# vkit-x/vkit

Hardware: AMD Instinct MI355X
Metric: Mpixels/s (2048^2 RGB, geo+photo chain) (higher is better)
Workload: dtype u8; 1 GPU; C3 fused chain: camera_cubic_curve remap (level 5) + gaussian_blur(sigma=1.0) + color_shift(37) + gaussion_noise(std=10.0, the numpy stream default_rng(5000 + i) drawn on the device inside every step), states built from the configs inside every step, 2048x2048x3 uint8, batch 256 per GPU; batch_per_gpu=256, image=2048x2048x3, noise_mode=tiles, states=built on the device from the configs inside every step (vkx_camera_states_dev), lanes=1

## Files before the change

### vkit_amd/csrc/fused.hip

```cpp
#include "vkx_internal.h"
#include "vkx_cell.h"
#include "vkx_color.h"

#include <float.h>
#include <memory>
#include <stdlib.h>
#include <string.h>

namespace {

constexpr int W = 64;
constexpr int RMAX = 3;
constexpr int NLDSCELL = 64;
#ifndef VKX_FUSED_NWAVES
#define VKX_FUSED_NWAVES 8
#endif
constexpr int NWAVES = VKX_FUSED_NWAVES;
constexpr int NTHREADS = 64 * NWAVES;
constexpr int ROWS_PER_WAVE = 8;
constexpr int WH = NWAVES * ROWS_PER_WAVE;
__host__ __device__ constexpr int tile_side(int R) { return (W - 2 * R) & ~3; }
__host__ __device__ constexpr int tile_height(int R) { return WH == W ? tile_side(R) : WH - 2 * R; }
#ifndef VKX_FUSED_CGROUP
#define VKX_FUSED_CGROUP 2
// ... 198 lines not shown
    }
    double r = __builtin_amdgcn_rcp(sdx);
    double e = fma(-sdx, r, 1.0);
    r = fma(r, e, r);
    e = fma(-sdx, r, 1.0);
    r = fma(r, e, r);
    const double snx = __builtin_amdgcn_div_scale(nx, de, true, &fnx);
    const double sny = __builtin_amdgcn_div_scale(ny, de, true, &fny);
    const double px = snx * r, py = sny * r;
    const double ex = fma(-sdx, px, snx), ey = fma(-sdx, py, sny);
    qx = __builtin_amdgcn_div_fixup(__builtin_amdgcn_div_fmas(ex, r, px, fnx), de, nx);
    qy = __builtin_amdgcn_div_fixup(__builtin_amdgcn_div_fmas(ey, r, py, fny), de, ny);
}

__device__ __forceinline__ bool div_pair_f32_fast(double nx, double ny, double de, float &fx, float &fy)
{
    double r = __builtin_amdgcn_rcp(de);
    double e = fma(-de, r, 1.0);
    r = fma(r, e, r);
    e = fma(-de, r, 1.0);
    r = fma(r, e, r);
    const double qx = nx * r, qy = ny * r;
    const uint32_t lx = (uint32_t)__double_as_longlong(qx) & 0x1fffffffu, ly = (uint32_t)__double_as_longlong(qy) & 0x1fffffffu;
    const bool danger = (lx - (0x10000000u - 16u)) < 32u || (ly - (0x10000000u - 16u)) < 32u;
    fx = (float)qx;
    fy = (float)qy;
    return __builtin_amdgcn_ballot_w64(danger) == 0;
}

__device__ __forceinline__ void rim_sample_rgb(gsrc_t src, int sh, int sw, ptrdiff_t sstride, int X, int Y, uint32_t &prb, uint32_t &pg)
{
    const int sx = vkd::sat_short(X >> 5), sy = vkd::sat_short(Y >> 5);
    const int fx = X & 31, fy = Y & 31;
    prb = 0; pg = 0;
    if (sx >= sw || sx + 1 < 0 || sy >= sh || sy + 1 < 0) return;
    const bool x0 = sx >= 0, x1 = sx + 1 < sw, y0 = sy >= 0, y1 = sy + 1 < sh;
    const gsrc_t r0 = src + (ptrdiff_t)sy * sstride + (ptrdiff_t)sx * 3, r1 = r0 + sstride;
    const int w00 = (32 - fy) * (32 - fx), w01 = (32 - fy) * fx, w10 = fy * (32 - fx), w11 = fy * fx;
    uint32_t c[3];
#pragma unroll
    for (int k = 0; k < 3; k++) {
        const int v0 = (x0 && y0) ? r0[k] : 0;
        const int v1 = (x1 && y0) ? r0[3 + k] : 0;
        const int v2 = (x0 && y1) ? r1[k] : 0;
        const int v3 = (x1 && y1) ? r1[3 + k] : 0;
        c[k] = (uint32_t)(v0 * w00 + v1 * w01 + v2 * w10 + v3 * w11 + 512) >> 10;
    }
    prb = c[0] | (c[2] << 16);
    pg = c[1];
}

struct HsvLut {
    int sdiv[256];
    int hdiv[256];
};

__device__ __forceinline__ void hue_shift_px(const int *sdiv, const int *hdiv, int delta, int &r, int &g, int &b)
{
    int H, S, V;
    vkd::rgb2hsv_full<true>(sdiv, hdiv, r, g, b, H, S, V);
    H = (H + delta) & 255;
    vkd::hsv2rgb_full(H, S, V, r, g, b);
}

constexpr int P_ = 97;
constexpr int kPairPitch = 2 * P_;
constexpr size_t kLdsOwn = sizeof(uint32_t) * WH * P_;
constexpr size_t kLdsHbB = 1024;
constexpr size_t kLdsCellR = sizeof(CellR) * NLDSCELL;
constexpr size_t kLdsCellH = sizeof(double) * 9 * NLDSCELL;
constexpr size_t kLdsLut = sizeof(int) * 512;
constexpr size_t kLdsSel = sizeof(uint32_t) * 8;
constexpr size_t kLdsNoiseRows = sizeof(uint32_t) * 2 * WH;
constexpr size_t kFusedLds = kLdsOwn + kLdsHbB + kLdsCellR + kLdsCellH + kLdsLut + kLdsSel + 16 + kLdsNoiseRows;

typedef const double __attribute__((address_space(3))) *lds_cdouble_t;


__device__ __forceinline__ int cvt_i32_sat(float v)
{
    int r;
    asm("v_cvt_i32_f32 %0, %1" : "=v"(r) : "v"(v));
    return r;
}

template <int KIND, bool STREAK = false, int RC = -1>
__device__ __forceinline__ void chain_tile(const ItemDev &it, const int tx, const int ty,
                                           const vkc::CellC *__restrict__ cells, const TileBin &bin,
                                           const HsvLut *__restrict__ lut, int phase_limit, const ElemPack *els = nullptr)
{
    constexpr bool INTERIOR = KIND == 1, EMPTY = KIND == 2;
    extern __shared__ __attribute__((aligned(16))) unsigned char smem[];
    uint32_t *own = (uint32_t *)smem;
    uint16_t *hbB = (uint16_t *)(smem + kLdsOwn);
    CellR *lcr = (CellR *)(smem + kLdsOwn + kLdsHbB);
    double *lch = (double *)(smem + kLdsOwn + kLdsHbB + kLdsCellR);
    int *lsdiv = (int *)(smem + kLdsOwn + kLdsHbB + kLdsCellR + kLdsCellH);
    int *lhdiv = lsdiv + 256;
    uint32_t *lsel = (uint32_t *)(lhdiv + 256);
    int *lflag = (int *)(lsel + 8);
    uint32_t *lnrow = (uint32_t *)(smem + kLdsOwn + kLdsHbB + kLdsCellR + kLdsCellH + kLdsLut + kLdsSel + 16);

    const int tid = threadIdx.x, lane = tid & 63, wave = __builtin_amdgcn_readfirstlane(tid >> 6);
    const int R = RC >= 0 ? RC : it.R, K = 2 * R + 1, Tw = tile_side(R), Th = tile_height(R);
    const int dw = it.dw, dh = it.dh;
    const int x0 = tx * Tw, y0 = ty * Th;
    const int tw = INTERIOR ? Tw : min(Tw, dw - x0), th = INTERIOR ? Th : min(Th, dh - y0);
    const int wx0 = x0 - R, wy0 = y0 - R;
    const int cx0 = INTERIOR ? wx0 : max(wx0, 0), cx1 = INTERIOR ? wx0 + W : min(wx0 + W, dw);
    const int cy0 = INTERIOR ? wy0 : max(wy0, 0), cy1 = INTERIOR ? wy0 + WH : min(wy0 + WH, dh);

    const gsrc_t src = (gsrc_t)it.src;
    const ptrdiff_t sstride = it.sstride;
    const int sh = it.sh, sw = it.sw;

    const int ocx = lane - R;
    const bool ocol = ocx >= 0 && ocx < tw;
    const int r0 = bin.rmin, c0 = bin.cmin;
    const int nr = max(0, bin.rmax1 - bin.rmin), ncol = max(0, bin.cmax1 - bin.cmin);
    const int nc = bin.rmax1 > 0 ? nr * ncol : 0;
    const int cw = it.cols - 1;
    const vkc::CellC *gcell = cells + it.cell_base;

    constexpr int kRecPerLane = NLDSCELL / (NTHREADS / 16);
    static_assert(NLDSCELL == kRecPerLane * (NTHREADS / 16), "whole records per lane and chunk");
    const float rcp_ncol = __builtin_amdgcn_rcpf((float)max(ncol, 1));
    auto chunk_fetch = [&](int base, int cn_, unsigned long long (&v)[kRecPerLane]) {
#pragma unroll
        for (int h = 0; h < kRecPerLane; h++) {
            const int rec = (tid >> 4) + h * (NTHREADS / 16);
            v[h] = 0;
            if (rec < cn_) {
                const int k = base + rec;
                const int rr = div_small(k, ncol, rcp_ncol), cc = k - rr * ncol;
                const unsigned long long VKX_GLOBAL *s8 =
                    (const unsigned long long VKX_GLOBAL *)(gcell + (r0 + rr) * cw + (c0 + cc));
                v[h] = s8[tid & 15];
            }
        }
    };
    auto chunk_store = [&](int cn_, const unsigned long long (&v)[kRecPerLane]) {
#pragma unroll
        for (int h = 0; h < kRecPerLane; h++) {
            const int rec = (tid >> 4) + h * (NTHREADS / 16), part = tid & 15;
            if (rec < cn_) {
                if (part < 8) ((unsigned long long *)(lch + rec * 9))[part] = v[h];
                else if (part < 15) ((unsigned long long *)(lcr + rec))[part - 8] = v[h];
            }
        }
    };
    auto load_chunk = [&](int base, int cn_) {
        unsigned long long v[kRecPerLane];
        chunk_fetch(base, cn_, v);
        chunk_store(cn_, v);
    };

    typedef uint32_t u32x2 __attribute__((ext_vector_type(2)));
    u32x2 nrec = {0u, 0u};
    const bool nrows_here = !(KIND == 3) && wave < WH / 64 && it.noise_rows != nullptr;
    const int nrow_y = wave * 64 + lane;
    if (nrows_here && nrow_y < th)
        nrec = ((const u32x2 VKX_GLOBAL *)it.noise_rows)[(size_t)(y0 + nrow_y) * (size_t)it.tiles_x + (size_t)tx];

    uint32_t kq[2 * RMAX + 1];
#pragma unroll
    for (int i = 0; i < 2 * RMAX + 1; i++) kq[i] = (R > 0 && i < K) ? it.kq[i < K - 1 - i ? i : K - 1 - i] : 0;
// ... 298 lines not shown
                ta[u] = 0; tb[u] = 0;
                if (fast[u]) {
                    const uint32_t o0 = __umul24((uint32_t)sy, (uint32_t)sstride) + __umul24((uint32_t)sx, 3u);
                    ta[u] = *(const u64_u1 VKX_GLOBAL *)(src + (size_t)o0);
                    tb[u] = *(const u64_u1 VKX_GLOBAL *)(src + (size_t)(o0 + (uint32_t)sstride));
                }
            }
            uint32_t prb[CGROUP], pg[CGROUP];
#pragma unroll
            for (int u = 0; u < CGROUP; u++) {
                prb[u] = 0; pg[u] = 0;
                if (!rowok[u]) continue;
                if (colok) {
                    const int fx = X[u] & 31, fy = Y[u] & 31;
                    if (fast[u]) {
                        const uint32_t wx = (uint32_t)(32 - fx) | ((uint32_t)fx << 24);
                        const uint32_t t0 = (uint32_t)ta[u], t1 = (uint32_t)(ta[u] >> 32), b0 = (uint32_t)tb[u], b1 = (uint32_t)(tb[u] >> 32);
                        const uint32_t ar = __builtin_amdgcn_udot4(t0, wx, 0u, false);
                        const uint32_t ag = __builtin_amdgcn_udot4(__builtin_amdgcn_alignbyte(t1, t0, 1), wx, 0u, false);
                        const uint32_t ab = __builtin_amdgcn_udot4(__builtin_amdgcn_alignbyte(t1, t0, 2), wx, 0u, false);
                        const uint32_t br = __builtin_amdgcn_udot4(b0, wx, 0u, false);
                        const uint32_t bg = __builtin_amdgcn_udot4(__builtin_amdgcn_alignbyte(b1, b0, 1), wx, 0u, false);
                        const uint32_t bb = __builtin_amdgcn_udot4(__builtin_amdgcn_alignbyte(b1, b0, 2), wx, 0u, false);
                        const uint32_t wy0 = (uint32_t)(32 - fy), wy1 = (uint32_t)fy;
                        const uint32_t r = mad_u24(br, wy1, mad_u24_cs(ar, wy0, 512u)) >> 10;
                        const uint32_t g = mad_u24(bg, wy1, mad_u24_cs(ag, wy0, 512u)) >> 10;
                        const uint32_t b = mad_u24(bb, wy1, mad_u24_cs(ab, wy0, 512u)) >> 10;
                        prb[u] = r | (b << 16);
                        pg[u] = g;
                    } else {
                        rim_sample_rgb(src, sh, sw, sstride, X[u], Y[u], prb[u], pg[u]);
                    }
                }
            }
            static_assert(CGROUP == 2, "phase D works on the window-row pair of one iteration");
            const int ly0 = wave * ROWS_PER_WAVE + g0;
            if (!(rowok[0] || rowok[1])) continue;
            if (R > 0) {
                const uint32_t gg = pg[0] | (pg[1] << 16);
                uint32_t a0 = 0, a1 = 0, ag = 0;
#pragma unroll
                for (int i = 0; i < 2 * RMAX + 1; i++) {
                    if (i < K) {
                        uint32_t v0 = prb[0], v1 = prb[1], vg = gg;
                        if (!(INTERIOR && RC >= 0 && i == RC)) {
                            v0 = (uint32_t)__builtin_amdgcn_ds_bpermute(srcl[i], (int)prb[0]);
                            v1 = (uint32_t)__builtin_amdgcn_ds_bpermute(srcl[i], (int)prb[1]);
                            vg = (uint32_t)__builtin_amdgcn_ds_bpermute(srcl[i], (int)gg);
                        }
                        a0 = mad_u24_ks(kq[i], v0, a0);
                        a1 = mad_u24_ks(kq[i], v1, a1);
                        ag = mad_u24_ks(kq[i], vg, ag);
                    }
                }
                uint32_t *pl = own + ly0 * P_ + lane;
                pl[0] = __builtin_amdgcn_perm(a1, a0, 0x05040100u);
                pl[64] = ag;
                pl[128] = __builtin_amdgcn_perm(a1, a0, 0x07060302u);
            } else {
#pragma unroll
                for (int u = 0; u < CGROUP; u++)
                    if (rowok[u]) own[(ly0 + u) * P_ + lane] = (prb[u] & 0xffu) | (pg[u] << 8) | (prb[u] & 0xff0000u);
            }
        }
        if constexpr (KIND == 3) return;
        __syncthreads();
        if (phase_limit == 2) return;

    }

    const ItemDev VKX_GLOBAL *ite_ = (const ItemDev VKX_GLOBAL *)&it;
    asm volatile("" : "+s"(ite_));
    const ItemDev VKX_GLOBAL &ite = *ite_;
    const gdst_t dst = (gdst_t)uniform64((uint64_t)ite.dst);
    const int16_t VKX_GLOBAL *noise = (const int16_t VKX_GLOBAL *)uniform64((uint64_t)ite.noise);
    const ptrdiff_t dstride = (ptrdiff_t)uniform64((uint64_t)ite.dstride), nstride = (ptrdiff_t)uniform64((uint64_t)ite.nstride);
    uint32_t nzA[ROWS_PER_WAVE];
    uint32_t nzB[ROWS_PER_WAVE];
    const bool tiled = noise && __builtin_amdgcn_readfirstlane(ite.noise_tiled) != 0;
    if constexpr (EMPTY) {
        if (nrows_here) *(u32x2 *)(lnrow + 2 * nrow_y) = nrec;
        if (tiled) __syncthreads();
    }
    const uint32_t k3 = (uint32_t)(ocx * 3);
    u32x2 nrow = {0u, 0u};
    if (tiled) nrow = *(const u32x2 *)(lnrow + 2 * (wave + NWAVES * (lane & 7)));
#pragma unroll
    for (int i = 0; i < ROWS_PER_WAVE; i++) {
        nzA[i] = 0; nzB[i] = 0;
        const int cy = wave + NWAVES * i;
        if (noise && ocol && cy < th) {
            const int16_t VKX_GLOBAL *np_;
            if (tiled) {
                const int16_t VKX_GLOBAL *rowp = noise + (size_t)(uint32_t)__builtin_amdgcn_readlane((int)nrow.x, i);
                const uint32_t sd = (uint32_t)__builtin_amdgcn_readlane((int)nrow.y, i);
                uint32_t off = k3;
                if ((sd & 0xffffu) < 3u * W) {
                    asm volatile("" ::: "memory");
                    off += k3 >= (sd & 0xffffu) ? (uint32_t)((int)sd >> 16) : 0u;
                }
                np_ = rowp + off;
            } else {
                np_ = noise + (ptrdiff_t)(y0 + cy) * nstride + (ptrdiff_t)(x0 + ocx) * 3;
            }
            nzA[i] = *(const u32_u1 VKX_GLOBAL *)np_;
            nzB[i] = *(const u16_u1 VKX_GLOBAL *)(np_ + 2);
        }
    }
    uint32_t wpair[RMAX + 1];
#pragma unroll
    for (int q = 0; q <= RMAX; q++) {
        const uint32_t e0 = 2 * q < K ? kq[2 * q < 2 * RMAX + 1 ? 2 * q : 0] : 0u, e1 = 2 * q + 1 < K ? kq[2 * q + 1 < 2 * RMAX + 1 ? 2 * q + 1 : 0] : 0u;
        const uint32_t o0 = (q > 0 && 2 * q - 1 < K) ? kq[q > 0 ? 2 * q - 1 : 0] : 0u, o1 = 2 * q < K ? kq[2 * q < 2 * RMAX + 1 ? 2 * q : 0] : 0u;
        wpair[q] = (wave & 1) ? (o0 | (o1 << 16)) : (e0 | (e1 << 16));
    }
    const bool hue_on = __builtin_amdgcn_readfirstlane(ite.hue_on) != 0;
    const int hue_delta = __builtin_amdgcn_readfirstlane(ite.hue_delta);
    const int right4 = min(lane + 1, 63) << 2;
    const uint32_t dcol4 = (uint32_t)(x0 * 3 + (ocx >> 2) * 12 + (ocx & 3) * 4);
    const int full4 = (tw >> 2) << 2;
    const bool streak_on = STREAK && ite.streak_on != 0;
    const int sxm = streak_on ? (x0 + ocx) % ite.streak_step : 0;
    const int sxd = streak_on ? (x0 + ocx) % ite.streak_dash_step : 0;
    uint32_t epx = 0;
    if constexpr (EMPTY) {
        int er = src[0], eg = src[1], eb = src[2];
        if (hue_on) hue_shift_px(lut->sdiv, lut->hdiv, hue_delta, er, eg, eb);
        epx = (uint32_t)er | ((uint32_t)eg << 8) | ((uint32_t)eb << 16);
    }
#pragma unroll
    for (int i = 0; i < ROWS_PER_WAVE; i++) {
        const int cy = wave + NWAVES * i;
        if (cy >= th) continue;
        const int gy = y0 + cy;
        uint32_t P = epx;
        if constexpr (!EMPTY) {
            if (R > 0) {
                int r, g, b;
                if constexpr (INTERIOR && RC > 0) {
                    const uint32_t *pl = own + (cy & ~1) * P_ + lane;
                    uint32_t ar = 32768u, ag = 32768u, ab = 32768u;
#pragma unroll
                    for (int q = 0; q <= RC; q++) {
                        ar = dot2_u16_ks(wpair[q], pl[q * kPairPitch], ar);
                        ag = dot2_u16_ks(wpair[q], pl[q * kPairPitch + 64], ag);
                        ab = dot2_u16_ks(wpair[q], pl[q * kPairPitch + 128], ab);
                    }
                    r = (int)(ar >> 16); g = (int)(ag >> 16); b = (int)(ab >> 16);
                } else {
                    uint32_t a0 = 0, a1 = 0, a2 = 0;
#pragma unroll
                    for (int j = 0; j < 2 * RMAX + 1; j++) {
                        if (j < K) {
                            const int yy = INTERIOR ? cy + j : vkd::reflect101(gy + j - R, dh) - wy0;
                            const uint16_t *h16 = (const uint16_t *)(own + (yy & ~1) * P_ + lane) + (yy & 1);
                            a0 += __umul24(kq[j], (uint32_t)h16[0]);
                            a1 += __umul24(kq[j], (uint32_t)h16[128]);
                            a2 += __umul24(kq[j], (uint32_t)h16[256]);
                        }
                    }
                    r = (int)((a0 + 32768u) >> 16); g = (int)((a1 + 32768u) >> 16); b = (int)((a2 + 32768u) >> 16);
                }
                if (phase_limit == 20) {
                    const int yy = INTERIOR ? cy + R : vkd::reflect101(gy, dh) - wy0;
                    const uint16_t *h16 = (const uint16_t *)(own + (yy & ~1) * P_ + lane) + (yy & 1);
                    r = h16[0] >> 8; g = h16[128] >> 8; b = h16[256] >> 8;
                }
                if (hue_on) P = vkd::hue_shift_packed(lsdiv, lhdiv, lsel, hue_delta, r, g, b);
                else P = (uint32_t)r | ((uint32_t)g << 8) | ((uint32_t)b << 16);
            } else {
                P = own[(cy + R) * P_ + lane];
                if (hue_on) P = vkd::hue_shift_packed(lsdiv, lhdiv, lsel, hue_delta, (int)(P & 0xff), (int)((P >> 8) & 0xff),
                                                      (int)((P >> 16) & 0xff));
            }
        }
        if (noise || (STREAK && streak_on)) {
            int r = (int)(P & 0xff), g = (int)((P >> 8) & 0xff), b = (int)((P >> 16) & 0xff);
            if (noise) {
                r = vkd::clamp_u8(r + (int)(int16_t)(nzA[i] & 0xffff));
                g = vkd::clamp_u8(g + (int)(int16_t)(nzA[i] >> 16));
                b = vkd::clamp_u8(b + (int)(int16_t)(nzB[i] & 0xffff));
            }
            if (STREAK && streak_on) {
                const int ym = gy % ite.streak_step, yd = gy % ite.streak_dash_step;
                bool mv = ite.streak_vert && sxm < ite.streak_thickness;
                bool mh = ite.streak_hori && ym < ite.streak_thickness;
                if (ite.streak_dash) {
                    if (yd < ite.streak_dash_gap) mv = false;
                    if (sxd < ite.streak_dash_gap) mh = false;
                }
                const float w1 = ite.streak_alpha, w0 = 1.0f - w1;
                int *ch[3] = {&r, &g, &b};
#pragma unroll
                for (int c = 0; c < 3; c++) {
                    int v = *ch[c];
                    const int col = ite.streak_color[c];
                    if (mv) { const float t0 = w0 * (float)v, t1 = w1 * (float)col; v = ite.streak_copy ? col : (int)(uint8_t)(t0 + t1); }
                    if (mh) { const float t0 = w0 * (float)v, t1 = w1 * (float)col; v = ite.streak_copy ? col : (int)(uint8_t)(t0 + t1); }
                    *ch[c] = v;
                }
            }
            P = (uint32_t)r | ((uint32_t)g << 8) | ((uint32_t)b << 16);
        }
        const uint32_t Pn = (uint32_t)__builtin_amdgcn_ds_bpermute(right4, (int)P);
        gdst_t drow = dst + (ptrdiff_t)gy * dstride + (ptrdiff_t)x0 * 3;
        if (ocol) {
            const int m = ocx & 3;
            if (INTERIOR || ocx < full4) {
                if (m < 3) {
                    const uint32_t wv = (P >> (8 * m)) | (Pn << (24 - 8 * m));
                    const uint32_t off = (uint32_t)gy * (uint32_t)dstride + dcol4;
                    *(u32_u1 VKX_GLOBAL *)(dst + (size_t)off) = wv;
                }
            } else {
                gdst_t d = drow + ocx * 3;
                d[0] = (uint8_t)P; d[1] = (uint8_t)(P >> 8); d[2] = (uint8_t)(P >> 16);
            }
        }
    }
}

template <bool STREAK>
__global__ void __launch_bounds__(NTHREADS, VKX_FUSED_WAVES_PER_EU) k_chain_fused(const ItemDev *__restrict__ items,
                                                          const vkc::CellC *__restrict__ cells,
                                                          const TileBin *__restrict__ bins,
                                                          const HsvLut *__restrict__ lut, int phase_limit)
{
    const int slots = gridDim.x;
    const ItemDev &it = items[blockIdx.y];
    const int ntiles = it.tiles_x * it.tiles_y;
    const int per = (ntiles + 7) >> 3;
    const int run = (int)((blockIdx.x + blockIdx.y) & 7), pos = (int)(blockIdx.x >> 3);
    const int tl = run * per + pos;
    if (pos >= per || tl >= ntiles) return;
    if (phase_limit == 10) return;
    const int tile_id = (int)blockIdx.y * slots + tl;
    const TileBin bin = bins[tile_id];
    const int ty = __builtin_amdgcn_readfirstlane(div_small(tl, it.tiles_x, __builtin_amdgcn_rcpf((float)it.tiles_x)));
    const int tx = tl - ty * it.tiles_x;
    const int Tw = tile_side(it.R), Th = tile_height(it.R);
    const int wx0 = tx * Tw - it.R, wy0 = ty * Th - it.R;
    const int nc = bin.rmax1 > 0 ? max(0, bin.rmax1 - bin.rmin) * max(0, bin.cmax1 - bin.cmin) : 0;
    const bool interior = wx0 >= 0 && wy0 >= 0 && wx0 + W <= it.dw && wy0 + WH <= it.dh && nc <= NLDSCELL && phase_limit != 3;
#ifdef VKX_FUSED_CENSUS
    (void)interior;
    chain_tile<1, STREAK, VKX_FUSED_CENSUS>(it, tx, ty, cells, bin, lut, phase_limit);
    return;
#endif
    if (nc == 0) chain_tile<2, STREAK>(it, tx, ty, cells, bin, lut, phase_limit);
    else if (interior) {
        switch (it.R) {
        case 0: chain_tile<1, STREAK, 0>(it, tx, ty, cells, bin, lut, phase_limit); break;
        case 1: chain_tile<1, STREAK, 1>(it, tx, ty, cells, bin, lut, phase_limit); break;
        case 2: chain_tile<1, STREAK, 2>(it, tx, ty, cells, bin, lut, phase_limit); break;
        default: chain_tile<1, STREAK, 3>(it, tx, ty, cells, bin, lut, phase_limit); break;
        }
    } else {
        switch (it.R) {
        case 0: chain_tile<0, STREAK, 0>(it, tx, ty, cells, bin, lut, phase_limit); break;
        case 1: chain_tile<0, STREAK, 1>(it, tx, ty, cells, bin, lut, phase_limit); break;
        case 2: chain_tile<0, STREAK, 2>(it, tx, ty, cells, bin, lut, phase_limit); break;
        default: chain_tile<0, STREAK, 3>(it, tx, ty, cells, bin, lut, phase_limit); break;
        }
    }
}

__global__ void __launch_bounds__(NTHREADS, 8) k_tile_remap(const ItemDev *__restrict__ items,
                                                           const vkc::CellC *__restrict__ cells,
                                                           const TileBin *__restrict__ bins, const ElemPack pack)
{
    const int slots = gridDim.x;
    const ItemDev &it = items[blockIdx.y];
    const int ntiles = it.tiles_x * it.tiles_y;
    const int per = (ntiles + 7) >> 3;
    const int run = (int)((blockIdx.x + blockIdx.y) & 7), pos = (int)(blockIdx.x >> 3);
    const int tl = run * per + pos;
    if (pos >= per || tl >= ntiles) return;
    const int tile_id = (int)blockIdx.y * slots + tl;
    const TileBin bin = bins[tile_id];
    const int ty = __builtin_amdgcn_readfirstlane(div_small(tl, it.tiles_x, __builtin_amdgcn_rcpf((float)it.tiles_x)));
    const int tx = tl - ty * it.tiles_x;
    chain_tile<3>(it, tx, ty, cells, bin, nullptr, 0, &pack);
}

__global__ void __launch_bounds__(256) k_chain_noise_rows(const ItemDev *__restrict__ items)
{
    typedef uint32_t u32x2 __attribute__((ext_vector_type(2)));
    const ItemDev &it = items[blockIdx.y];
    if (!it.noise_rows) return;
    const uint32_t k = blockIdx.x * 256u + threadIdx.x;
    if (k >= (uint32_t)it.dh * (uint32_t)it.tiles_x) return;
    const uint32_t y = k / (uint32_t)it.tiles_x, tx = k - y * (uint32_t)it.tiles_x;
    const u32x2 VKX_GLOBAL *tab = (const u32x2 VKX_GLOBAL *)it.noise_table;
// ... 311 lines not shown
```

### vkit_amd/csrc/nprand.hip

```cpp
#include "vkx_internal.h"
#include "np_ziggurat.h"

#include <string.h>
#include <algorithm>

namespace {

typedef unsigned __int128 u128;
#define VKX_GLOBAL __attribute__((address_space(1)))

#ifndef VKX_NP_ROUNDS
#define VKX_NP_ROUNDS 48
#endif
constexpr int kRounds = VKX_NP_ROUNDS;
static_assert(kRounds % 2 == 0 && kRounds >= 2 && kRounds <= 64, "rounds per tile");
constexpr int kTile = 64 * kRounds;
constexpr double kNorR = 3.6541528853610087963519472518;
constexpr double kNorInvR = 0.27366123732975827203338247596;

#define PCG_MULT ((((u128)0x2360ED051FC65DA4ull) << 64) | (u128)0x4385DF649FCCF645ull)

struct JumpTabs {
    uint64_t pow2[64][4];
    uint64_t lane[64][4];
// ... 593 lines not shown
}

constexpr int kInlineJobs = 8;
struct NpJobPack { NpJob jobs[kInlineJobs]; };

template <bool INLINE>
__global__ void __launch_bounds__(256) k_np_tile_states(const NpJob *__restrict__ jobs_dev, NpJobPack pack, int n_jobs, long long total_tiles,
                                                        uint64_t *__restrict__ states , NpJob *__restrict__ jobs_out,
                                                        vkx_np_result *__restrict__ results, unsigned *__restrict__ done,
                                                        const NpTabs *__restrict__ tabs)
{
    const NpJob *jobs = INLINE ? pack.jobs : jobs_dev;
    if (blockIdx.x == 0) {
        if (INLINE) {
            const uint32_t *src = (const uint32_t *)pack.jobs;
            uint32_t *dst = (uint32_t *)jobs_out;
            for (unsigned i = threadIdx.x; i < (unsigned)n_jobs * (sizeof(NpJob) / 4); i += 256) dst[i] = src[i];
        }
        uint32_t *r = (uint32_t *)results;
        for (unsigned i = threadIdx.x; i < (unsigned)n_jobs * (sizeof(vkx_np_result) / 4); i += 256) r[i] = 0;
        if (threadIdx.x == 0) *done = 0;
    }
    const JumpTabs &g_jump = tabs->jump;
    const long long tile = (long long)blockIdx.x * 256 + threadIdx.x;
    if (tile >= total_tiles) return;
    const NpJob &job = jobs[job_of_tile(jobs, n_jobs, tile)];
    unsigned long long d = (unsigned long long)(tile - job.tile_base) * kTile;
    u128 s = mk128(job.state);
    const u128 inc = mk128(job.inc);
    for (int i = 0; d; i++, d >>= 1)
        if (d & 1) s = mk128(&g_jump.pow2[i][0]) * s + mk128(&g_jump.pow2[i][2]) * inc;
    states[2 * tile] = (uint64_t)s;
    states[2 * tile + 1] = (uint64_t)(s >> 64);
}

__device__ __forceinline__ void np_results_out(unsigned *done, const vkx_np_result *results, vkx_np_result *results_host, int n_jobs)
{
    if (!results_host) return;
    __shared__ bool s_last;
    asm volatile("s_waitcnt vmcnt(0)" ::: "memory");
    __syncthreads();
    if (threadIdx.x == 0) s_last = atomicAdd(done, 1u) == gridDim.x - 1;
    __syncthreads();
    if (!s_last) return;
    const uint32_t *src = (const uint32_t *)results;
    uint32_t *dst = (uint32_t *)results_host;
    for (unsigned i = threadIdx.x; i < (unsigned)n_jobs * (sizeof(vkx_np_result) / 4); i += blockDim.x)
        dst[i] = __hip_atomic_load(src + i, __ATOMIC_RELAXED, __HIP_MEMORY_SCOPE_AGENT);
}

template <class Emit>
__global__ void __launch_bounds__(256) k_np_draw(const NpJob *__restrict__ jobs, int n_jobs, long long total_tiles,
                                                 const uint64_t *__restrict__ states, TileInfo *__restrict__ info,
                                                 typename Emit::Store *__restrict__ rec_val, uint64_t *__restrict__ rec_mask,
                                                 vkx_np_result *__restrict__ results, const NpTabs *__restrict__ tabs)
{
    __shared__ uint4 zig[256];
    __shared__ double fi[256];
    __shared__ WaveWork<typename Emit::Store, false> work[4];
    load_tables(zig, fi, tabs);
    const JumpTabs &g_jump = tabs->jump;
    const long long n_waves = (long long)gridDim.x * 4;
    for (long long tile = (long long)blockIdx.x * 4 + (threadIdx.x >> 6); tile < total_tiles; tile += n_waves) {
        const int j = job_of_tile(jobs, n_jobs, tile);
        const NpJob &job = jobs[j];
        uint32_t count, carry, flags = 0;
        uint64_t start0, emit0;
        bool has_tail;
        u128 s, s2;
        tile_lane_states(g_jump, job, mk128(&states[2 * tile]), s, s2);
        walk_tile<Emit, kRecord>(job, g_jump, zig, fi, work[threadIdx.x >> 6], s, s2, 0u, 0, 0,
                                 (typename Emit::Store VKX_GLOBAL *)(rec_val + tile * kTile), (uint64_t VKX_GLOBAL *)(rec_mask + tile * kRounds),
                                 nullptr, count, carry, start0, emit0, has_tail, flags, nullptr);
        if (__lane_id() == 0) {
            TileInfo t;
            t.count0 = count; t.out0 = carry | (has_tail ? 0x80000000u : 0u); t.start0 = start0; t.emit0 = emit0;
            info[tile] = t;
        }
        if (flags) atomicOr(&results[j].flags, flags);
    }
}

constexpr int kSlot = kTile + 16;
#ifndef VKX_NP_DRAW_WAVES
#define VKX_NP_DRAW_WAVES 8
#endif
constexpr int kDrawWaves = VKX_NP_DRAW_WAVES;

template <class Emit>
__global__ void __launch_bounds__(64 * kDrawWaves) k_np_draw_compact(const NpJob *__restrict__ jobs, int n_jobs, long long total_tiles,
                                                                    long long run, const uint64_t *__restrict__ states, TileInfo *__restrict__ info,
                                                                    vkx_np_result *__restrict__ results, const NpTabs *__restrict__ tabs)
{
    struct Lds {
        uint4 zig[256];
        double fi[256];
        WaveWork<int16_t, true> work[kDrawWaves];
    };
    __shared__ Lds lds;
    uint4 *zig = lds.zig;
    double *fi = lds.fi;
    WaveWork<int16_t, true> *work = lds.work;
    load_tables(zig, fi, tabs);
    const JumpTabs &g_jump = tabs->jump;
    const long long wave = (long long)blockIdx.x * kDrawWaves + __builtin_amdgcn_readfirstlane((int)(threadIdx.x >> 6));
    const long long run_end = min(total_tiles, (wave + 1) * run);
    int j = 0;
    long long job_end = 0;
    u128 s = 0, s2 = 0;
    for (long long tile = wave * run; tile < run_end; tile++) {
        if (tile >= job_end) {
            j = job_of_tile(jobs, n_jobs, tile);
            job_end = jobs[j].tile_base + jobs[j].n_tiles;
            tile_lane_states(g_jump, jobs[j], mk128(&states[2 * tile]), s, s2);
        }
        const NpJob &job = jobs[j];
        uint32_t count, carry, flags = 0;
        uint64_t start0, emit0;
        bool has_tail;
        walk_tile<Emit, kCompact>(job, g_jump, zig, fi, work[threadIdx.x >> 6], s, s2, 0u, 0, 0,
                                  (int16_t VKX_GLOBAL *)(job.rec + (tile - job.tile_base) * kSlot), nullptr, nullptr,
                                  count, carry, start0, emit0, has_tail, flags, nullptr);
        if (__lane_id() == 0) {
            TileInfo t;
            t.count0 = count; t.out0 = carry | (has_tail ? 0x80000000u : 0u); t.start0 = start0; t.emit0 = emit0;
            info[tile] = t;
        }
        if (flags) atomicOr(&results[j].flags, flags);
    }
}

__global__ void __launch_bounds__(1024) k_np_resolve(const NpJob *__restrict__ jobs, const uint64_t *__restrict__ states,
                                                     const TileInfo *__restrict__ info_all, TilePlan *__restrict__ plan_all,
                                                     vkx_np_result *__restrict__ results, const NpTabs *__restrict__ tabs)
{
    __shared__ uint4 zig[256];
    __shared__ double fi[256];
    __shared__ WaveWork<int16_t, false> work[1];
    __shared__ unsigned long long part[1024];
    __shared__ uint32_t n_irregular;
    extern __shared__ uint64_t irregular[];
    const NpJob &job = jobs[blockIdx.x];
    const int T = job.n_tiles;
    const TileInfo *info = info_all + job.tile_base;
    TilePlan *plan = plan_all + job.tile_base;
    const uint64_t *st = states + 2 * job.tile_base;
    const int words = (T + 63) >> 6;
    if (threadIdx.x == 0) n_irregular = 0;
    load_tables(zig, fi, tabs);
    const JumpTabs &g_jump = tabs->jump;
    for (int w = threadIdx.x >> 6; w < words; w += 16) {
        const int j = w * 64 + (threadIdx.x & 63);
        bool bad = false;
        if (j < T) {
            const uint32_t c = j ? (info[j - 1].out0 & 0x7fffffffu) : 0u;
            const TileInfo t = info[j];
            const bool ok = c < 64 && ((t.start0 >> c) & 1);
            TilePlan p;
            p.prefix = 0;
            p.c_in = c;
            p.count = ok ? t.count0 - (uint32_t)__builtin_popcountll(t.emit0 & ((1ull << c) - 1)) : 0u;
            plan[j] = p;
            bad = !ok;
        }
        const uint64_t m = __ballot(bad);
        if ((threadIdx.x & 63) == 0) {
// ... 286 lines not shown
    };
#pragma unroll 4
    for (uint32_t i = 0; i < (uint32_t)kTile / 256; i++) {
        if (64u * i >= body) break;
        const uint32_t g = lane + 64u * i;
        if (g < body) {
            const uint32_t e = head + 4u * g;
            const unsigned long long nz = *(const u64_u2 VKX_GLOBAL *)(rec + e);
            if (ADD) {
                const uint32_t px = *(const uint32_t VKX_GLOBAL *)((const uint8_t VKX_GLOBAL *)src + prefix + e);
                pk16 lo = __builtin_bit_cast(pk16, __builtin_amdgcn_perm(0u, px, 0x0c010c00u));
                pk16 hi = __builtin_bit_cast(pk16, __builtin_amdgcn_perm(0u, px, 0x0c030c02u));
                lo += __builtin_bit_cast(pk16, (uint32_t)nz);
                hi += __builtin_bit_cast(pk16, (uint32_t)(nz >> 32));
                const pk16 zero = {0, 0}, top = {255, 255};
                lo = __builtin_elementwise_min(__builtin_elementwise_max(lo, zero), top);
                hi = __builtin_elementwise_min(__builtin_elementwise_max(hi, zero), top);
                *(uint32_t VKX_GLOBAL *)((uint8_t VKX_GLOBAL *)dst + prefix + e) =
                    __builtin_amdgcn_perm(__builtin_bit_cast(uint32_t, hi), __builtin_bit_cast(uint32_t, lo), 0x06040200u);
            } else {
                *(unsigned long long VKX_GLOBAL *)((int16_t VKX_GLOBAL *)dst + prefix + e) = nz;
            }
        }
    }
    if (lane < 8) {
        const uint32_t k = lane & 3u;
        if (lane < 4 ? k < head : k < tail) one(lane < 4 ? k : head + 4u * body + k);
    }
}

template <bool ADD>
__global__ void __launch_bounds__(256) k_np_apply(const NpJob *__restrict__ jobs, int n_jobs, long long total_tiles,
                                                  const TileInfo *__restrict__ info, const TilePlan *__restrict__ plan)
{
    const long long tile = (long long)blockIdx.x * 4 + (threadIdx.x >> 6);
    if (tile >= total_tiles) return;
    const TilePlan p = plan[tile];
    const uint64_t emit0 = info[tile].emit0;
    const NpJob &job = jobs[job_of_tile(jobs, n_jobs, tile)];
    const long long prefix = (long long)rfl64(p.prefix);
    if (prefix >= job.n) return;
    TilePlan pu;
    pu.prefix = (unsigned long long)prefix;
    pu.c_in = (uint32_t)__builtin_amdgcn_readfirstlane((int)p.c_in);
    pu.count = (uint32_t)__builtin_amdgcn_readfirstlane((int)p.count);
    if (tile_needs_walk(job, pu, 0u, false)) return;
    const uint32_t skip = (uint32_t)__builtin_popcountll(rfl64(emit0) & ((1ull << pu.c_in) - 1));
    apply_tile<ADD>((const int16_t VKX_GLOBAL *)job.rec + (tile - job.tile_base) * kSlot + skip, prefix, pu.count, job.src, job.dst);
}

__global__ void __launch_bounds__(256) k_np_tiles_expand(const uint2 *__restrict__ table, const int16_t *__restrict__ slots, int n_tiles,
                                                         long long n, int16_t *__restrict__ dst)
{
    const int t = (int)(blockIdx.x * 4 + (threadIdx.x >> 6));
    if (t >= n_tiles) return;
    const uint2 a = table[t], b = table[t + 1];
    const long long prefix = (long long)__builtin_amdgcn_readfirstlane((int)a.x) & 0xffffffffLL;
    const uint32_t next = (uint32_t)__builtin_amdgcn_readfirstlane((int)b.x), skip = (uint32_t)__builtin_amdgcn_readfirstlane((int)a.y);
    if (prefix >= n) return;
    uint32_t count = next - (uint32_t)prefix;
    if (prefix + count > n) count = (uint32_t)(n - prefix);
    apply_tile<false>((const int16_t VKX_GLOBAL *)slots + (long long)t * kSlot + skip, prefix, count, nullptr, dst);
}

__global__ void __launch_bounds__(256) k_np_tiles_finish(const NpJob *__restrict__ jobs, const TileInfo *__restrict__ info,
                                                         const TilePlan *__restrict__ plan)
{
    const NpJob &job = jobs[blockIdx.y];
    const long long t = (long long)blockIdx.x * 256 + threadIdx.x;
    if (t >= job.n_tiles) return;
    const long long tile = job.tile_base + t;
    auto skip_of = [&](long long tl, const TilePlan &p) -> uint32_t {
        if ((long long)p.prefix < job.n && tile_needs_walk(job, p, 0u, false)) return 0u;
        if (p.c_in & kIrregular) return 0u;
        return (uint32_t)__builtin_popcountll(info[tl].emit0 & ((1ull << p.c_in) - 1));
    };
    const TilePlan p = plan[tile];
    const uint32_t skip = skip_of(tile, p);
    job.table[t] = make_uint2((uint32_t)p.prefix, skip);
    int16_t *rec = job.rec + t * kSlot;
    if (t + 1 < job.n_tiles) {
        const TilePlan pn = plan[tile + 1];
        const int16_t *nxt = rec + kSlot + skip_of(tile + 1, pn);
        rec[skip + p.count] = nxt[0];
        rec[skip + p.count + 1] = nxt[1];
    } else {
        job.table[t + 1] = make_uint2((uint32_t)(p.prefix + p.count), 0u);
        uint32_t *header = (uint32_t *)job.table - 4;
        header[0] = (uint32_t)job.n_tiles;
        header[1] = (uint32_t)kSlot;
        *(unsigned long long *)(header + 2) = p.prefix + p.count;
    }
}

template <class Emit, bool TILES = false, int STEP = 64>
__global__ void __launch_bounds__(64) k_np_place_walk(const NpJob *__restrict__ jobs, int n_jobs, long long total_tiles,
                                                       const uint64_t *__restrict__ states, const TileInfo *__restrict__ info,
                                                       const TilePlan *__restrict__ plan, vkx_np_result *__restrict__ results,
                                                       unsigned *__restrict__ done, vkx_np_result *__restrict__ results_host,
                                                       const NpTabs *__restrict__ tabs)
{
    __shared__ uint4 zig[256];
    __shared__ double fi[256];
    __shared__ __attribute__((aligned(16))) WaveWork<typename Emit::Store, true> work[1];
    load_tables(zig, fi, tabs);
    const JumpTabs &g_jump = tabs->jump;
    const int lane = __lane_id();
    const long long n_waves = (long long)gridDim.x;
    for (long long t0 = (long long)blockIdx.x * STEP; t0 < total_tiles; t0 += n_waves * STEP) {
        const long long mine = t0 + lane;
        bool want = false;
        if (lane < STEP && mine < total_tiles) {
            const NpJob &jb = jobs[job_of_tile(jobs, n_jobs, mine)];
            const TilePlan p = plan[mine];
            want = (long long)p.prefix < jb.n && tile_needs_walk(jb, p, info[mine].out0, Emit::kCheckAtStore);
        }
        uint64_t todo = __ballot(want);
        while (todo) {
            const int b = __builtin_ctzll(todo);
            todo &= todo - 1;
            const long long tile = t0 + b;
            const int j = job_of_tile(jobs, n_jobs, tile);
            const NpJob &job = jobs[j];
            const TilePlan p = plan[tile];
            uint32_t count, carry, flags = 0;
            uint64_t start0, emit0;
            bool ht;
            void *dst = job.dst;
            if (TILES) dst = (void *)((intptr_t)(job.rec + (tile - job.tile_base) * kSlot) - 2 * (intptr_t)p.prefix);
            u128 s, s2;
            tile_lane_states(g_jump, job, mk128(&states[2 * tile]), s, s2);
            walk_tile<Emit, kEmit>(job, g_jump, zig, fi, work[0], s, s2, p.c_in & ~kIrregular,
                                   (long long)p.prefix, (tile - job.tile_base) * kTile, nullptr, nullptr, dst, count, carry, start0, emit0, ht,
                                   flags, &results[j].draws);
            if (flags) atomicOr(&results[j].flags, flags);
        }
    }
    np_results_out(done, results, results_host, n_jobs);
}

__global__ void __launch_bounds__(256) k_np_choice_impulse(const NpJob *__restrict__ jobs, int n_jobs, long long total_tiles,
                                                           const uint64_t *__restrict__ states, vkx_np_result *__restrict__ results,
                                                           unsigned *__restrict__ done, vkx_np_result *__restrict__ results_host,
                                                           const NpTabs *__restrict__ tabs)
{
    const JumpTabs &g_jump = tabs->jump;
    const long long n_waves = (long long)gridDim.x * 4;
    const int lane = __lane_id();
    for (long long tile = (long long)blockIdx.x * 4 + (threadIdx.x >> 6); tile < total_tiles; tile += n_waves) {
        const int jb = job_of_tile(jobs, n_jobs, tile);
        const NpJob &job = jobs[jb];
        if (tile == job.tile_base && lane == 0) {
            __hip_atomic_store(&results[jb].draws, (unsigned long long)job.n, __ATOMIC_RELAXED, __HIP_MEMORY_SCOPE_AGENT);
            __hip_atomic_store(&results[jb].samples, (unsigned long long)job.n, __ATOMIC_RELAXED, __HIP_MEMORY_SCOPE_AGENT);
        }
        const u128 inc = mk128(job.inc), a64 = mk128(g_jump.a64), c64 = mk128(job.c64);
        u128 s = mk128(&g_jump.lane[lane][0]) * mk128(&states[2 * tile]) + mk128(&g_jump.lane[lane][2]) * inc;
        const long long e0 = (tile - job.tile_base) * kTile + lane;
        const int cn = job.cn;
#pragma unroll 1
        for (int r = 0; r < kRounds; r++) {
            const long long e = e0 + 64 * r;
            if (e - lane >= job.n) break;
            const double u = u2dbl(pcg_out(s));
            if (e < job.n) {
                const int sel = (job.cdf[0] <= u) + (job.cdf[1] <= u) + (job.cdf[2] <= u);
                uint8_t *d = (uint8_t *)job.dst + e * cn;
                if (job.kind == VKX_NP_CHOICE3_U8) {
// ... 458 lines not shown
```

Measured before the change: 70930 Mpixels/s.

## Load noise as 4-byte groups and apply with packed saturating adds at store

For lanes writing grouped 4-byte output words, the noise for the same four bytes is now fetched as one 8-byte load and added to the packed output word with packed 16-bit adds and v_sat_pk_u8_i16, skipping the per-channel unpack and clamp. Every fourth lane no longer loads noise. The noise record compaction now lends three samples from the next tile instead of two, so the overlapping 8-byte reads stay inside valid data at tile seams. It reduces scalar ALU work and load instructions in the noise step, at the cost of coupling the noise table layout to the output grouping.

```diff
diff --git a/vkit_amd/csrc/fused.hip b/vkit_amd/csrc/fused.hip
--- a/vkit_amd/csrc/fused.hip
+++ b/vkit_amd/csrc/fused.hip
@@ -304,6 +304,19 @@
     int r;
     asm("v_cvt_i32_f32 %0, %1" : "=v"(r) : "v"(v));
     return r;
+}
+
+__device__ __forceinline__ uint32_t add_noise_u8x4(uint32_t px, uint32_t n01, uint32_t n23)
+{
+    typedef unsigned short pk16 __attribute__((ext_vector_type(2)));
+    pk16 lo = __builtin_bit_cast(pk16, __builtin_amdgcn_perm(px, px, 0x0c010c00u));
+    pk16 hi = __builtin_bit_cast(pk16, __builtin_amdgcn_perm(px, px, 0x0c030c02u));
+    lo += __builtin_bit_cast(pk16, n01);
+    hi += __builtin_bit_cast(pk16, n23);
+    uint32_t lo8, hi8;
+    asm("v_sat_pk_u8_i16 %0, %1" : "=v"(lo8) : "v"(__builtin_bit_cast(uint32_t, lo)));
+    asm("v_sat_pk_u8_i16 %0, %1" : "=v"(hi8) : "v"(__builtin_bit_cast(uint32_t, hi)));
+    return __builtin_amdgcn_perm(hi8, lo8, 0x05040100u);
 }
 
 template <int KIND, bool STREAK = false, int RC = -1>
@@ -768,14 +781,18 @@
         if (nrows_here) *(u32x2 *)(lnrow + 2 * nrow_y) = nrec;
         if (tiled) __syncthreads();
     }
-    const uint32_t k3 = (uint32_t)(ocx * 3);
+    const int full4 = (tw >> 2) << 2;
+    const bool grouped = !STREAK && (INTERIOR || ocx < full4);
+    const uint32_t g4 = (uint32_t)((ocx >> 2) * 12 + (ocx & 3) * 4);
+    const uint32_t k3 = grouped ? g4 : (uint32_t)(ocx * 3);
+    const bool nlane = ocol && !(grouped && (ocx & 3) == 3);
     u32x2 nrow = {0u, 0u};
     if (tiled) nrow = *(const u32x2 *)(lnrow + 2 * (wave + NWAVES * (lane & 7)));
 #pragma unroll
     for (int i = 0; i < ROWS_PER_WAVE; i++) {
         nzA[i] = 0; nzB[i] = 0;
         const int cy = wave + NWAVES * i;
-        if (noise && ocol && cy < th) {
+        if (noise && nlane && cy < th) {
             const int16_t VKX_GLOBAL *np_;
             if (tiled) {
                 const int16_t VKX_GLOBAL *rowp = noise + (size_t)(uint32_t)__builtin_amdgcn_readlane((int)nrow.x, i);
@@ -787,10 +804,16 @@
                 }
                 np_ = rowp + off;
             } else {
-                np_ = noise + (ptrdiff_t)(y0 + cy) * nstride + (ptrdiff_t)(x0 + ocx) * 3;
-            }
-            nzA[i] = *(const u32_u1 VKX_GLOBAL *)np_;
-            nzB[i] = *(const u16_u1 VKX_GLOBAL *)(np_ + 2);
+                np_ = noise + (ptrdiff_t)(y0 + cy) * nstride + (ptrdiff_t)x0 * 3 + (ptrdiff_t)k3;
+            }
+            if (grouped) {
+                const unsigned long long v = *(const u64_u1 VKX_GLOBAL *)np_;
+                nzA[i] = (uint32_t)v;
+                nzB[i] = (uint32_t)(v >> 32);
+            } else {
+                nzA[i] = *(const u32_u1 VKX_GLOBAL *)np_;
+                nzB[i] = *(const u16_u1 VKX_GLOBAL *)(np_ + 2);
+            }
         }
     }
     uint32_t wpair[RMAX + 1];
@@ -803,8 +826,7 @@
     const bool hue_on = __builtin_amdgcn_readfirstlane(ite.hue_on) != 0;
     const int hue_delta = __builtin_amdgcn_readfirstlane(ite.hue_delta);
     const int right4 = min(lane + 1, 63) << 2;
-    const uint32_t dcol4 = (uint32_t)(x0 * 3 + (ocx >> 2) * 12 + (ocx & 3) * 4);
-    const int full4 = (tw >> 2) << 2;
+    const uint32_t dcol4 = (uint32_t)(x0 * 3) + g4;
     const bool streak_on = STREAK && ite.streak_on != 0;
     const int sxm = streak_on ? (x0 + ocx) % ite.streak_step : 0;
     const int sxd = streak_on ? (x0 + ocx) % ite.streak_dash_step : 0;
@@ -860,12 +882,12 @@
                                                       (int)((P >> 16) & 0xff));
             }
         }
-        if (noise || (STREAK && streak_on)) {
+        if ((STREAK || !INTERIOR) && ((noise && !grouped) || (STREAK && streak_on))) {
             int r = (int)(P & 0xff), g = (int)((P >> 8) & 0xff), b = (int)((P >> 16) & 0xff);
             if (noise) {
-                r = vkd::clamp_u8(r + (int)(int16_t)(nzA[i] & 0xffff));
-                g = vkd::clamp_u8(g + (int)(int16_t)(nzA[i] >> 16));
-                b = vkd::clamp_u8(b + (int)(int16_t)(nzB[i] & 0xffff));
+                r = vkd::clamp_u8((int)(int16_t)(r + (int)(nzA[i] & 0xffff)));
+                g = vkd::clamp_u8((int)(int16_t)(g + (int)(nzA[i] >> 16)));
+                b = vkd::clamp_u8((int)(int16_t)(b + (int)(nzB[i] & 0xffff)));
             }
             if (STREAK && streak_on) {
                 const int ym = gy % ite.streak_step, yd = gy % ite.streak_dash_step;
@@ -894,7 +916,8 @@
             const int m = ocx & 3;
             if (INTERIOR || ocx < full4) {
                 if (m < 3) {
-                    const uint32_t wv = (P >> (8 * m)) | (Pn << (24 - 8 * m));
+                    uint32_t wv = (P >> (8 * m)) | (Pn << (24 - 8 * m));
+                    if (!STREAK && noise) wv = add_noise_u8x4(wv, nzA[i], nzB[i]);
                     const uint32_t off = (uint32_t)gy * (uint32_t)dstride + dcol4;
                     *(u32_u1 VKX_GLOBAL *)(dst + (size_t)off) = wv;
                 }
diff --git a/vkit_amd/csrc/nprand.hip b/vkit_amd/csrc/nprand.hip
--- a/vkit_amd/csrc/nprand.hip
+++ b/vkit_amd/csrc/nprand.hip
@@ -699,6 +699,7 @@
 }
 
 constexpr int kSlot = kTile + 16;
+constexpr int kLent = 3;
 #ifndef VKX_NP_DRAW_WAVES
 #define VKX_NP_DRAW_WAVES 8
 #endif
@@ -1151,8 +1152,9 @@
     if (t + 1 < job.n_tiles) {
         const TilePlan pn = plan[tile + 1];
         const int16_t *nxt = rec + kSlot + skip_of(tile + 1, pn);
-        rec[skip + p.count] = nxt[0];
-        rec[skip + p.count + 1] = nxt[1];
+        static_assert(kLent <= 16 && kSlot >= kTile + kLent, "a slot has room for its tile's samples and the lent ones");
+#pragma unroll
+        for (int k = 0; k < kLent; k++) rec[skip + p.count + k] = nxt[k];
     } else {
         job.table[t + 1] = make_uint2((uint32_t)(p.prefix + p.count), 0u);
         uint32_t *header = (uint32_t *)job.table - 4;
```

Result: faster. 71780 Mpixels/s, median of 6 (+1.2%).
